# bryanlimy/tf2-cyclegan

Hardware: AMD Instinct MI355X
Metric: images/sec (whole node) horse2zebra 256×256 (higher is better)
Workload: dtype bf16; 1 GPU; model=cyclegan-resnet9-patchgan, global_batch=4, per_gpu_batch=4, image_size=256, parallelism=dp1

## Files before the change

cyclegan_amd/ops/_hip/bind.cpp:

```cpp
#include <torch/extension.h>

namespace cyg {
at::Tensor conv2d_fwd(at::Tensor, at::Tensor, c10::optional<at::Tensor>,
                      int64_t, int64_t, int64_t, int64_t, int64_t, bool,
                      int64_t, double);
at::Tensor convt2d_fwd(at::Tensor, at::Tensor, c10::optional<at::Tensor>,
                       int64_t, int64_t, int64_t, int64_t, int64_t, int64_t,
                       double);
std::vector<at::Tensor> conv2d_fwd_stats(at::Tensor, at::Tensor,
                                         c10::optional<at::Tensor>, int64_t,
                                         int64_t, int64_t, int64_t, int64_t,
                                         bool, int64_t, double);
std::vector<at::Tensor> convt2d_fwd_stats(at::Tensor, at::Tensor,
                                          c10::optional<at::Tensor>, int64_t,
                                          int64_t, int64_t, int64_t, int64_t,
                                          int64_t, double);
at::Tensor conv2d_dgrad(at::Tensor, at::Tensor, int64_t, int64_t, int64_t,
                        int64_t, int64_t, int64_t, int64_t, bool);
at::Tensor convt2d_dgrad(at::Tensor, at::Tensor, int64_t, int64_t, int64_t,
                         int64_t, int64_t);
at::Tensor conv2d_wgrad(at::Tensor, at::Tensor, int64_t, int64_t, int64_t,
                        int64_t, int64_t, bool);
void conv2d_wgrad_into(at::Tensor, at::Tensor, int64_t, int64_t, int64_t,
                       int64_t, int64_t, bool, at::Tensor, bool, bool);
void fold_packed_dw_into(at::Tensor, at::Tensor, bool);
at::Tensor mfma_probe(at::Tensor, at::Tensor);
at::Tensor mx_probe(at::Tensor, at::Tensor, int64_t, int64_t);
at::Tensor mx_probe16(at::Tensor, at::Tensor, int64_t, int64_t);
at::Tensor glds_probe(at::Tensor, at::Tensor);
at::Tensor tr_probe(int64_t);
at::Tensor quant_fp8(at::Tensor, at::Tensor);
at::Tensor quant_fp8_d(at::Tensor, at::Tensor, at::Tensor);
void amax_roll(at::Tensor, int64_t);
at::Tensor conv2d_fp8_fwd(at::Tensor, at::Tensor, at::Tensor,
                          c10::optional<at::Tensor>, c10::optional<at::Tensor>,
                          int64_t, int64_t, int64_t, int64_t, int64_t, bool, int64_t, double);
std::vector<at::Tensor> conv2d_fp8_fwd_stats(
    at::Tensor, at::Tensor, at::Tensor, c10::optional<at::Tensor>,
    c10::optional<at::Tensor>, int64_t, int64_t, int64_t, int64_t, int64_t,
    bool, int64_t, double);
std::vector<at::Tensor> instnorm_fwd(at::Tensor, at::Tensor, at::Tensor,
                                     double, int64_t, double,
                                     c10::optional<at::Tensor>,
                                     c10::optional<at::Tensor>,
                                     c10::optional<at::Tensor>, int64_t);
std::vector<at::Tensor> instnorm_fwd_q8(at::Tensor, at::Tensor, at::Tensor,
                                        double, int64_t, double,
                                        c10::optional<at::Tensor>,
                                        c10::optional<at::Tensor>,
                                        c10::optional<at::Tensor>, int64_t,
                                        at::Tensor, at::Tensor);
std::vector<at::Tensor> instnorm_bwd(at::Tensor, at::Tensor, at::Tensor,
                                     at::Tensor, at::Tensor,
                                     c10::optional<at::Tensor>, int64_t,
                                     double, c10::optional<at::Tensor>,
                                     c10::optional<at::Tensor>,
                                     c10::optional<at::Tensor>, bool);
at::Tensor act_bwd(at::Tensor, at::Tensor, int64_t, double);
at::Tensor channel_sum(at::Tensor, c10::optional<at::Tensor>, bool);
at::Tensor reflect_pad_fwd(at::Tensor, int64_t, int64_t, int64_t, int64_t);
at::Tensor reflect_pad_bwd(at::Tensor, int64_t, int64_t, int64_t, int64_t);
at::Tensor persample_loss_fwd(at::Tensor, at::Tensor, bool);
at::Tensor persample_loss_const_fwd(at::Tensor, double, bool);
std::vector<at::Tensor> persample_loss_bwd(at::Tensor, at::Tensor, at::Tensor,
                                           bool, bool, bool);
at::Tensor persample_loss_const_bwd(at::Tensor, double, at::Tensor, bool);
void adam_step_dev(at::Tensor, at::Tensor, at::Tensor, at::Tensor, at::Tensor,
                   double, double, double);
void adam_ema_step(at::Tensor, at::Tensor, at::Tensor, at::Tensor, at::Tensor,
                   double, double, double, double, int64_t, double);
void adam_ema_step_dev(at::Tensor, at::Tensor, at::Tensor, at::Tensor,
                       at::Tensor, at::Tensor, double, double, double, double);
void shadow_gather(at::Tensor, at::Tensor, at::Tensor);
void shadow_fold(at::Tensor, at::Tensor, at::Tensor);
void fold_upconv_dw_into(at::Tensor, at::Tensor, bool, bool);
void adam_step(at::Tensor, at::Tensor, at::Tensor, at::Tensor, double, double,
               double, double, int64_t);
at::Tensor augment_batch(at::Tensor, at::Tensor, at::Tensor, int64_t, int64_t,
                         at::Tensor);
at::Tensor pool_exchange(at::Tensor, at::Tensor, at::Tensor, at::Tensor);
std::vector<at::Tensor> ssim_fwd(at::Tensor, at::Tensor, int64_t);
at::Tensor ssim_bwd(at::Tensor, at::Tensor, at::Tensor, at::Tensor, at::Tensor,
                    at::Tensor);
}

PYBIND11_MODULE(TORCH_EXTENSION_NAME, m) {
  m.def("conv2d_fwd", &cyg::conv2d_fwd);
  m.def("convt2d_fwd", &cyg::convt2d_fwd);
  m.def("conv2d_fwd_stats", &cyg::conv2d_fwd_stats);
  m.def("convt2d_fwd_stats", &cyg::convt2d_fwd_stats);
  m.def("conv2d_dgrad", &cyg::conv2d_dgrad);
  m.def("convt2d_dgrad", &cyg::convt2d_dgrad);
  m.def("conv2d_wgrad", &cyg::conv2d_wgrad);
  m.def("conv2d_wgrad_into", &cyg::conv2d_wgrad_into, py::arg("x"),
        py::arg("dy"), py::arg("kh"), py::arg("kw"), py::arg("stride"),
        py::arg("pt"), py::arg("pl"), py::arg("reflect"), py::arg("out"),
        py::arg("accumulate"), py::arg("transpose_oi") = false);
  m.def("fold_packed_dw_into", &cyg::fold_packed_dw_into, py::arg("dwp"),
        py::arg("out"), py::arg("accumulate"));
  m.def("mfma_probe", &cyg::mfma_probe);
  m.def("mx_probe", &cyg::mx_probe);
  m.def("mx_probe16", &cyg::mx_probe16);
  m.def("glds_probe", &cyg::glds_probe);
  m.def("tr_probe", &cyg::tr_probe);
  m.def("quant_fp8", &cyg::quant_fp8);
  m.def("quant_fp8_d", &cyg::quant_fp8_d);
  m.def("amax_roll", &cyg::amax_roll);
  m.def("conv2d_fp8_fwd", &cyg::conv2d_fp8_fwd);
  m.def("conv2d_fp8_fwd_stats", &cyg::conv2d_fp8_fwd_stats);
  m.def("instnorm_fwd", &cyg::instnorm_fwd, py::arg("x"), py::arg("gamma"),
        py::arg("beta"), py::arg("eps"), py::arg("act"), py::arg("slope"),
        py::arg("residual"), py::arg("psum") = py::none(),
        py::arg("psq") = py::none(), py::arg("nslabs") = 0);
  m.def("instnorm_fwd_q8", &cyg::instnorm_fwd_q8, py::arg("x"),
        py::arg("gamma"), py::arg("beta"), py::arg("eps"), py::arg("act"),
        py::arg("slope"), py::arg("residual"), py::arg("psum"),
        py::arg("psq"), py::arg("nslabs"), py::arg("amax_prev"),
        py::arg("amax_cur"));
  m.def("instnorm_bwd", &cyg::instnorm_bwd, py::arg("dy"), py::arg("x"),
        py::arg("gamma"), py::arg("mean"), py::arg("rstd"), py::arg("yact"),
        py::arg("act"), py::arg("slope"), py::arg("beta") = py::none(),
        py::arg("dgamma_out") = py::none(), py::arg("dbeta_out") = py::none(),
        py::arg("accumulate") = false);
  m.def("act_bwd", &cyg::act_bwd);
  m.def("channel_sum", &cyg::channel_sum, py::arg("x"),
        py::arg("out") = py::none(), py::arg("accumulate") = false);
  m.def("reflect_pad_fwd", &cyg::reflect_pad_fwd);
  m.def("reflect_pad_bwd", &cyg::reflect_pad_bwd);
  m.def("persample_loss_fwd", &cyg::persample_loss_fwd);
  m.def("persample_loss_const_fwd", &cyg::persample_loss_const_fwd);
  m.def("persample_loss_bwd", &cyg::persample_loss_bwd);
  m.def("persample_loss_const_bwd", &cyg::persample_loss_const_bwd);
  m.def("adam_step", &cyg::adam_step);
  m.def("adam_step_dev", &cyg::adam_step_dev);
  m.def("adam_ema_step", &cyg::adam_ema_step);
  m.def("adam_ema_step_dev", &cyg::adam_ema_step_dev);
  m.def("shadow_gather", &cyg::shadow_gather);
  m.def("shadow_fold", &cyg::shadow_fold);
  m.def("fold_upconv_dw_into", &cyg::fold_upconv_dw_into, py::arg("dv"),
        py::arg("out"), py::arg("accumulate"), py::arg("transposed"));
  m.def("augment_batch", &cyg::augment_batch);
  m.def("pool_exchange", &cyg::pool_exchange);
  m.def("ssim_fwd", &cyg::ssim_fwd, py::arg("y_true"), py::arg("y_pred"),
        py::arg("save_maps") = 0);
  m.def("ssim_bwd", &cyg::ssim_bwd, py::arg("x"), py::arg("y"), py::arg("am"),
        py::arg("bm"), py::arg("cm"), py::arg("dout"));
}
```

cyclegan_amd/ops/_hip/conv.hip:

```cpp

#include <torch/extension.h>
#include <ATen/cuda/CUDAContext.h>

#include "common.h"

namespace cyg {

constexpr int BM = 128, BN = 64, BK = 64;
constexpr int NTHREADS = 256;
constexpr int LDK = BK + 8;

struct ConvParams {
  const short* __restrict__ x;
  const short* __restrict__ w;
  const short* __restrict__ bias;
  short* __restrict__ y;
  int B, H, W, Cin, OH, OW, Cout, KH, KW;
  int stride, pt, pl;
  int reflect;
  int act;  float slope;
  const float* dq;
  const float* dqb;
  long M, KTOT;
  int mtiles, ntiles;
  float* psum;
  float* psq;
  int tps;
  long ringoff;
  int wt, wl, wH, wW;
};

DEV int ring_index(int qh, int qw, int OH, int OW, int wt, int wl, int wH,
                   int wW) {
  if (qh < wt) return qh * OW + qw;
  if (qh >= wt + wH) return (qh - wH) * OW + qw;
  return (OH - wH) * OW + (qh - wt) * (OW - wW) + (qw < wl ? qw : qw - wW);
}

DEV int xcd_chunk(int bid, int nb) {
  return (nb % 8 == 0) ? (bid % 8) * (nb / 8) + bid / 8 : bid;
}


template <bool IS_CONVT, bool ALIGNED, int STRIDE>
__global__ __launch_bounds__(NTHREADS) void conv_gemm_kernel(ConvParams p) {
  const int stride = STRIDE ? STRIDE : p.stride;
  __shared__ short As[BM][LDK];
  __shared__ short Bs[BN][LDK];
  __shared__ long rowxb[BM];
  __shared__ long rowyb[BM];
  __shared__ int rowih[BM], rowiw[BM];
  __shared__ char rowok[BM];

  const int tid = threadIdx.x;
  const int lane = tid & 63;
  const int wid = tid >> 6;
  const int bid = xcd_chunk(blockIdx.x, gridDim.x);
  const int mt = bid % p.mtiles, nt = bid / p.mtiles;
  const long m0 = (long)mt * BM;
  const int n0 = nt * BN;

  for (int r = tid; r < BM; r += NTHREADS) {
    long m = m0 + r;
    bool ok = m < p.M;
    long mm = ok ? m : 0;
    int ow = (int)(mm % p.OW);
    int oh = (int)((mm / p.OW) % p.OH);
    int b = (int)(mm / ((long)p.OW * p.OH));
    rowok[r] = ok;
    rowxb[r] = (long)b * p.H * p.W * p.Cin;
    rowyb[r] = ((long)(b * p.OH + oh) * p.OW + ow) * p.Cout;
    if (IS_CONVT) {
      rowih[r] = oh + p.pt;
      rowiw[r] = ow + p.pl;
    } else {
      rowih[r] = oh * stride - p.pt;
      rowiw[r] = ow * stride - p.pl;
    }
  }
  __syncthreads();

  v4f acc[4][2] = {};

  const int wr = wid >> 1, wc = wid & 1;
  const int wm0 = wr * 64, wn0 = wc * 32;
  const int fr = lane & 15;
  const int fg = lane >> 4;

  for (long k0 = 0; k0 < p.KTOT; k0 += BK) {
    if (ALIGNED) {
      #pragma unroll 2
      for (int c = tid; c < BM * (BK / 8); c += NTHREADS) {
        int row = c >> 3;
        int kc = (c & 7) * 8;
        long k = k0 + kc;
        v8s val = {};
        if (k < p.KTOT && rowok[row]) {
          int tap = (int)(k / p.Cin);
          int ci = (int)(k - (long)tap * p.Cin);
          int dkh = tap / p.KW, dkw = tap - (tap / p.KW) * p.KW;
          bool valid = true;
          int ih, iw;
          if (IS_CONVT) {
            int nh = rowih[row] - dkh, nw = rowiw[row] - dkw;
            valid = nh >= 0 && nw >= 0 && (nh % stride) == 0 &&
                    (nw % stride) == 0;
            ih = nh / stride; iw = nw / stride;
            valid = valid && ih < p.H && iw < p.W;
          } else {
            ih = rowih[row] + dkh; iw = rowiw[row] + dkw;
            if (p.reflect) {
              ih = mirror_idx(ih, p.H); iw = mirror_idx(iw, p.W);
            } else {
              valid = ih >= 0 && ih < p.H && iw >= 0 && iw < p.W;
            }
          }
          if (valid)
            val = *(const v8s*)(p.x + rowxb[row] + ((long)ih * p.W + iw) * p.Cin + ci);
        }
        *(v8s*)&As[row][kc] = val;
// ... 25 lines not shown
            }
          }
          if (valid)
            val = p.x[rowxb[row] + ((long)ih * p.W + iw) * p.Cin + ci];
        }
        As[row][kc] = val;
      }
    }

    if (ALIGNED) {
      #pragma unroll 2
      for (int c = tid; c < BN * (BK / 8); c += NTHREADS) {
        int n = c >> 3;
        int kc = (c & 7) * 8;
        long k = k0 + kc;
        v8s val = {};
        if (n0 + n < p.Cout && k < p.KTOT)
          val = *(const v8s*)(p.w + (long)(n0 + n) * p.KTOT + k);
        *(v8s*)&Bs[n][kc] = val;
      }
    } else {
      for (int c = tid; c < BN * BK; c += NTHREADS) {
        int n = c >> 6;
        int kc = c & 63;
        long k = k0 + kc;
        Bs[n][kc] = (n0 + n < p.Cout && k < p.KTOT)
                        ? p.w[(long)(n0 + n) * p.KTOT + k] : (short)0;
      }
    }
    __syncthreads();

    #pragma unroll
    for (int kk = 0; kk < BK; kk += 32) {
      v8bf a0 = *(const v8bf*)&As[wm0 + 0 * 16 + fr][kk + fg * 8];
      v8bf a1 = *(const v8bf*)&As[wm0 + 1 * 16 + fr][kk + fg * 8];
      v8bf a2 = *(const v8bf*)&As[wm0 + 2 * 16 + fr][kk + fg * 8];
      v8bf a3 = *(const v8bf*)&As[wm0 + 3 * 16 + fr][kk + fg * 8];
      v8bf b0 = *(const v8bf*)&Bs[wn0 + 0 * 16 + fr][kk + fg * 8];
      v8bf b1 = *(const v8bf*)&Bs[wn0 + 1 * 16 + fr][kk + fg * 8];
      acc[0][0] = __builtin_amdgcn_mfma_f32_16x16x32_bf16(a0, b0, acc[0][0], 0, 0, 0);
      acc[0][1] = __builtin_amdgcn_mfma_f32_16x16x32_bf16(a0, b1, acc[0][1], 0, 0, 0);
      acc[1][0] = __builtin_amdgcn_mfma_f32_16x16x32_bf16(a1, b0, acc[1][0], 0, 0, 0);
      acc[1][1] = __builtin_amdgcn_mfma_f32_16x16x32_bf16(a1, b1, acc[1][1], 0, 0, 0);
      acc[2][0] = __builtin_amdgcn_mfma_f32_16x16x32_bf16(a2, b0, acc[2][0], 0, 0, 0);
      acc[2][1] = __builtin_amdgcn_mfma_f32_16x16x32_bf16(a2, b1, acc[2][1], 0, 0, 0);
      acc[3][0] = __builtin_amdgcn_mfma_f32_16x16x32_bf16(a3, b0, acc[3][0], 0, 0, 0);
      acc[3][1] = __builtin_amdgcn_mfma_f32_16x16x32_bf16(a3, b1, acc[3][1], 0, 0, 0);
    }
    __syncthreads();
  }

  #pragma unroll
  for (int nf = 0; nf < 2; ++nf) {
    int n = n0 + wn0 + nf * 16 + fr;
    if (n >= p.Cout) continue;
    float bv = p.bias ? b2f(p.bias[n]) : 0.f;
    #pragma unroll
    for (int mf = 0; mf < 4; ++mf) {
      #pragma unroll
      for (int r = 0; r < 4; ++r) {
        int rl = wm0 + mf * 16 + fg * 4 + r;
        if (!rowok[rl]) continue;
        float v = apply_act(acc[mf][nf][r] + bv, p.act, p.slope);
        p.y[rowyb[rl] + n] = f2b(v);
      }
    }
  }
}


template <int BNT>
struct ConvSmemT {
  long rowyb[BM];
  int rowih[BM], rowiw[BM];
  unsigned rowxb[BM];
  char rowok[BM];
  char _pad[16 - (BM % 16 ? BM % 16 : 16)];
  short A[2][BM * BK];
  short Bt[2][BNT * BK];
};

constexpr int NW = 8;

template <bool IS_CONVT, int STRIDE, int BNT, bool PHASED = false>
__global__ __launch_bounds__(NW * 64) void conv_glds_kernel(ConvParams p) {
  constexpr int NT = NW * 64;
  constexpr int API = 16 / NW;
  constexpr int TBI = BNT / 8;
  constexpr int BPI = TBI >= NW ? TBI / NW : 1;
  constexpr int NF = BNT >= 32 ? 2 : 1;
  constexpr int NWC = BNT / (NF * 16);
  constexpr int NWR = NW / NWC;
  constexpr int MF = (BM / NWR) / 16;
  const int stride = STRIDE ? STRIDE : p.stride;
  extern __shared__ __attribute__((aligned(16))) char smem_raw[];
  auto& sm = *reinterpret_cast<ConvSmemT<BNT>*>(smem_raw);

  const int tid = threadIdx.x;
  const int lane = tid & 63;
  const int w = tid >> 6;
  const int bid = (IS_CONVT && STRIDE == 2)
                      ? blockIdx.x : xcd_chunk(blockIdx.x, gridDim.x);
  const int mt = bid % p.mtiles, nt = bid / p.mtiles;
  const int n0 = nt * BNT;

  static_assert(!PHASED || (IS_CONVT && STRIDE == 2), "PHASED");
  const int tpp = PHASED ? (p.mtiles >> 2) : 0;
  const int phase = PHASED ? mt / tpp : 0;
  const int phh = phase >> 1, phw = phase & 1;
  const int OH2 = p.OH >> 1, OW2 = p.OW >> 1;
  const long m0 = PHASED ? (long)(mt - phase * tpp) * BM : (long)mt * BM;
  const int nvh = PHASED ? ((p.KH - phh + 1) >> 1) : 0;
  const int nvw = PHASED ? ((p.KW - phw + 1) >> 1) : 0;
  const long KEFF = PHASED ? (long)nvh * nvw * p.Cin : p.KTOT;

  for (int r = tid; r < BM; r += NT) {
    if (PHASED) {
      long mp = m0 + r;
      long Mp = (long)p.B * OH2 * OW2;
      bool ok = mp < Mp;
      long mm = ok ? mp : 0;
      int owp = (int)(mm % OW2);
      int ohp = (int)((mm / OW2) % OH2);
      int b = (int)(mm / ((long)OW2 * OH2));
      int i = 2 * ohp + ((phh + p.pt) & 1);
      int j = 2 * owp + ((phw + p.pl) & 1);
      sm.rowok[r] = ok && i < p.OH && j < p.OW;
      sm.rowxb[r] = (unsigned)((long)b * p.H * p.W * p.Cin * 2);
      sm.rowyb[r] = ((long)(b * p.OH + i) * p.OW + j) * p.Cout;
      sm.rowih[r] = (i + p.pt - phh) >> 1;
      sm.rowiw[r] = (j + p.pl - phw) >> 1;
    } else {
      long m = m0 + r;
      bool ok = m < p.M;
      long mm = ok ? m : 0;
      int ow = (int)(mm % p.OW);
      int oh = (int)((mm / p.OW) % p.OH);
      int b = (int)(mm / ((long)p.OW * p.OH));
      sm.rowok[r] = ok;
      sm.rowxb[r] = (unsigned)((long)b * p.H * p.W * p.Cin * 2);
      long yb = ((long)(b * p.OH + oh) * p.OW + ow) * p.Cout;
      if (IS_CONVT && p.ringoff != 0) {
        const int i = oh - p.wt, j = ow - p.wl;
        if ((unsigned)i < (unsigned)p.wH && (unsigned)j < (unsigned)p.wW) {
          yb = (((long)b * p.wH + i) * p.wW + j) * p.Cout;
        } else {
          const long rp = (long)p.OH * p.OW - (long)p.wH * p.wW;
          yb = p.ringoff +
               (b * rp + ring_index(oh, ow, p.OH, p.OW, p.wt, p.wl, p.wH,
                                    p.wW)) * p.Cout;
        }
      }
      sm.rowyb[r] = yb;
      if (IS_CONVT) {
        sm.rowih[r] = oh + p.pt;
        sm.rowiw[r] = ow + p.pl;
      } else {
        sm.rowih[r] = oh * stride - p.pt;
        sm.rowiw[r] = ow * stride - p.pl;
      }
    }
  }
  __syncthreads();

  const int lr = lane >> 3;
  const int klog = ((lane & 7) ^ lr) << 3;
  int aih[API], aiw[API];
  unsigned axb[API];
  bool aok[API];
  #pragma unroll
  for (int j = 0; j < API; ++j) {
    int r = (w * API + j) * 8 + lr;
    aih[j] = sm.rowih[r];
    aiw[j] = sm.rowiw[r];
    axb[j] = sm.rowxb[r];
    aok[j] = sm.rowok[r];
  }
  int bn[BPI];
  #pragma unroll
  for (int j = 0; j < BPI; ++j) bn[j] = (w * BPI + j) * 8 + lr + n0;
  const bool bw_on = w * BPI < TBI;
  static_assert(BNT == 16 || BNT == 64 || BNT == 128, "BNT");

  auto rx = __builtin_amdgcn_make_buffer_rsrc(
      (void*)p.x, 0, (unsigned)((long)p.B * p.H * p.W * p.Cin * 2), 0x00020000);
  auto rw = __builtin_amdgcn_make_buffer_rsrc(
      (void*)p.w, 0, (unsigned)(p.Cout * p.KTOT * 2), 0x00020000);

  const int nk = (int)((KEFF + BK - 1) / BK);
  const bool big_ci = p.Cin >= BK;

  long kcur;
  bool kv;
  int ci, dkh, dkw;
  unsigned avo[API];
  bool avalid[API];
  unsigned bvo[BPI];
  bool bnv[BPI];

  auto recompute_a = [&]() {
    #pragma unroll
    for (int j = 0; j < API; ++j) {
      avalid[j] = false;
      avo[j] = 0xFF000000u;
      if (!aok[j]) continue;
      bool valid = true;
      int ih, iw;
      if (PHASED) {
        ih = aih[j] - dkh; iw = aiw[j] - dkw;
        valid = ih >= 0 && iw >= 0 && ih < p.H && iw < p.W;
      } else if (IS_CONVT) {
        int nh = aih[j] - dkh, nw = aiw[j] - dkw;
        valid = nh >= 0 && nw >= 0 && (nh % stride) == 0 && (nw % stride) == 0;
        ih = nh / stride; iw = nw / stride;
        valid = valid && ih < p.H && iw < p.W;
      } else {
        ih = aih[j] + dkh; iw = aiw[j] + dkw;
        if (p.reflect) {
          ih = mirror_idx(ih, p.H); iw = mirror_idx(iw, p.W);
        } else {
          valid = ih >= 0 && ih < p.H && iw >= 0 && iw < p.W;
        }
      }
      if (valid) {
        avalid[j] = true;
        avo[j] = axb[j] + (unsigned)((((long)ih * p.W + iw) * p.Cin + ci) * 2);
      }
    }
  };

  auto recompute_b = [&]() {
    long kw_idx = kcur;
    if (PHASED)
      kw_idx = ((long)(2 * dkh + phh) * p.KW + (2 * dkw + phw)) * p.Cin + ci;
    #pragma unroll
    for (int j = 0; j < BPI; ++j)
      bvo[j] = (unsigned)(((long)bn[j] * p.KTOT + kw_idx) * 2);
  };

  auto decode_tap = [&]() {
    int tap = (int)(kcur / p.Cin);
    ci = (int)(kcur - (long)tap * p.Cin);
    if (PHASED) {
      dkh = tap / nvw;
      dkw = tap - dkh * nvw;
    } else {
      dkh = tap / p.KW;
      dkw = tap - dkh * p.KW;
    }
  };

  auto init_state = [&]() {
    kcur = klog;
    kv = kcur < KEFF;
    decode_tap();
    recompute_a();
    #pragma unroll
    for (int j = 0; j < BPI; ++j) bnv[j] = bn[j] < p.Cout;
    recompute_b();
  };

  auto advance = [&]() {
    kcur += BK;
    kv = kcur < KEFF;
    if (big_ci) {
      ci += BK;
      if (ci >= p.Cin) {
        ci -= p.Cin;
        if (PHASED) {
          if (++dkw == nvw) { dkw = 0; ++dkh; }
        } else {
          if (++dkw == p.KW) { dkw = 0; ++dkh; }
        }
        recompute_a();
        recompute_b();
      } else {
        #pragma unroll
        for (int j = 0; j < API; ++j) avo[j] += BK * 2;
        #pragma unroll
        for (int j = 0; j < BPI; ++j) bvo[j] += BK * 2;
      }
    } else {
      decode_tap();
      recompute_a();
      recompute_b();
    }
  };

  auto stage = [&](int buf) {
    #pragma unroll
    for (int j = 0; j < API; ++j) {
      unsigned vo = (kv && avalid[j]) ? avo[j] : 0xFF000000u;
      __builtin_amdgcn_raw_ptr_buffer_load_lds(
          rx, (__attribute__((address_space(3))) void*)&sm.A[buf][(w * API + j) * 512],
          16, vo, 0, 0, 0);
    }
    if (bw_on) {
      #pragma unroll
      for (int j = 0; j < BPI; ++j) {
        unsigned vo = (kv && bnv[j]) ? bvo[j] : 0xFF000000u;
        __builtin_amdgcn_raw_ptr_buffer_load_lds(
            rw, (__attribute__((address_space(3))) void*)&sm.Bt[buf][(w * BPI + j) * 512],
            16, vo, 0, 0, 0);
      }
    }
  };

  v4f acc[MF][NF] = {};
  const int wr = w / NWC, wc = w % NWC;
  const int wm0 = wr * (MF * 16), wn0 = wc * (NF * 16);
  const int fr = lane & 15;
  const int fg = lane >> 4;
  const int swz = (fr & 7) << 4;

  init_state();
  stage(0);
  __syncthreads();

  for (int kt = 0; kt < nk; ++kt) {
    if (kt + 1 < nk) {
      advance();
      stage((kt + 1) & 1);
    }
    const char* Ab = (const char*)sm.A[kt & 1];
    const char* Bb = (const char*)sm.Bt[kt & 1];
    #pragma unroll
    for (int kk = 0; kk < BK; kk += 32) {
      const int kbyte = (kk + fg * 8) * 2;
      v8bf a[MF], b[NF];
      #pragma unroll
      for (int mf = 0; mf < MF; ++mf)
        a[mf] = *(const v8bf*)(Ab + ((wm0 + mf * 16 + fr) << 7) + (kbyte ^ swz));
      #pragma unroll
      for (int nf = 0; nf < NF; ++nf)
        b[nf] = *(const v8bf*)(Bb + ((wn0 + nf * 16 + fr) << 7) + (kbyte ^ swz));
      #pragma unroll
      for (int mf = 0; mf < MF; ++mf)
        #pragma unroll
        for (int nf = 0; nf < NF; ++nf)
          acc[mf][nf] = __builtin_amdgcn_mfma_f32_16x16x32_bf16(
              a[mf], b[nf], acc[mf][nf], 0, 0, 0);
    }
    __syncthreads();
  }

  float cs[NF] = {}, cq[NF] = {};
  #pragma unroll
  for (int nf = 0; nf < NF; ++nf) {
    int n = n0 + wn0 + nf * 16 + fr;
    if (n >= p.Cout) continue;
    float bv = p.bias ? b2f(p.bias[n]) : 0.f;
    #pragma unroll
    for (int mf = 0; mf < MF; ++mf) {
      #pragma unroll
      for (int r = 0; r < 4; ++r) {
        int rl = wm0 + mf * 16 + fg * 4 + r;
// ... 1064 lines not shown
  if (q < nr * W) {
    i = span_nth(rs, q / W);
    j = q % W;
  } else {
    q -= nr * W;
    i = span_nth_out(rs, q / nc);
    j = span_nth(cs, q % nc);
  }
  int HP = H + pt + pb, WP = W + pl + pr;
  long rp = (long)HP * WP - (long)H * W;
  short* own = dx + (((long)b * H + i) * W + j) * C + g * 8;
  float s[8] = {};
  int hc[3] = {pt + i, pt - i, pt + 2 * (H - 1) - i};
  int wc_[3] = {pl + j, pl - j, pl + 2 * (W - 1) - j};
  #pragma unroll
  for (int a = 0; a < 3; ++a) {
    int qh = hc[a];
    if (qh < 0 || qh >= HP) continue;
    if (a > 0 && qh == hc[0]) continue;
    if (a == 2 && qh == hc[1]) continue;
    if (mirror_idx(qh - pt, H) != i) continue;
    #pragma unroll
    for (int d = 0; d < 3; ++d) {
      int qw = wc_[d];
      if (qw < 0 || qw >= WP) continue;
      if (d > 0 && qw == wc_[0]) continue;
      if (d == 2 && qw == wc_[1]) continue;
      if (mirror_idx(qw - pl, W) != j) continue;
      const short* src = (a == 0 && d == 0)
          ? own
          : ring + (b * rp + ring_index(qh, qw, HP, WP, pt, pl, H, W)) * C +
                g * 8;
      v8s v = *(const v8s*)src;
      #pragma unroll
      for (int e = 0; e < 8; ++e) s[e] += b2f(v[e]);
    }
  }
  v8s out;
  #pragma unroll
  for (int e = 0; e < 8; ++e) out[e] = f2b(s[e]);
  *(v8s*)own = out;
}


static inline int cdiv(long a, long b) { return (int)((a + b - 1) / b); }

static inline bool env_flag(const char* v) { return v && v[0] == '1'; }

static Span2 mirror_span(int n, int lo, int hi) {
  const int a0 = 1, b0 = std::min(lo, n - 1);
  const int a1 = std::max(n - 1 - hi, 0), b1 = n - 2;
  const int n0 = std::max(b0 - a0 + 1, 0), n1 = std::max(b1 - a1 + 1, 0);
  if (n0 == 0) return {a1, n1, a1 + n1, 0};
  if (n1 == 0) return {a0, n0, a0 + n0, 0};
  if (a1 <= a0 + n0) {
    const int a = std::min(a0, a1), b = std::max(b0, b1);
    return {a, b - a + 1, b + 1, 0};
  }
  return {a0, n0, a1, n1};
}

template <bool IS_CONVT, bool ALIGNED>
static void launch_conv_s(const ConvParams& p, dim3 grid, hipStream_t stream) {
  switch (p.stride) {
    case 1:
      hipLaunchKernelGGL((conv_gemm_kernel<IS_CONVT, ALIGNED, 1>), grid,
                         dim3(NTHREADS), 0, stream, p);
      break;
    case 2:
      hipLaunchKernelGGL((conv_gemm_kernel<IS_CONVT, ALIGNED, 2>), grid,
                         dim3(NTHREADS), 0, stream, p);
      break;
    default:
      hipLaunchKernelGGL((conv_gemm_kernel<IS_CONVT, ALIGNED, 0>), grid,
                         dim3(NTHREADS), 0, stream, p);
  }
}

static int conv_ntile(int Cout) {
  if (Cout <= 16) return 16;
  return (Cout % 128) == 0 ? 128 : 64;
}

template <bool IS_CONVT, int STRIDE, int BNT, bool PHASED = false>
static void launch_one_glds(const ConvParams& p, hipStream_t stream) {
  constexpr size_t SMB = sizeof(ConvSmemT<BNT>);
  static bool init = []() {
    hipFuncSetAttribute(
        (const void*)(conv_glds_kernel<IS_CONVT, STRIDE, BNT, PHASED>),
        hipFuncAttributeMaxDynamicSharedMemorySize, (int)SMB);
    return true;
  }();
  (void)init;
  hipLaunchKernelGGL((conv_glds_kernel<IS_CONVT, STRIDE, BNT, PHASED>),
                     dim3((long)p.mtiles * p.ntiles), dim3(NW * 64), SMB,
                     stream, p);
  hipError_t err = hipGetLastError();
  TORCH_CHECK(err == hipSuccess, "conv_glds launch failed (BNT=", BNT,
              " PHASED=", PHASED, "): ", hipGetErrorString(err));
}

template <bool IS_CONVT, int BNT>
static void launch_glds_s(const ConvParams& p, hipStream_t stream) {
  switch (p.stride) {
    case 1: launch_one_glds<IS_CONVT, 1, BNT>(p, stream); break;
    case 2: launch_one_glds<IS_CONVT, 2, BNT>(p, stream); break;
    default: launch_one_glds<IS_CONVT, 0, BNT>(p, stream);
  }
}

template <bool IS_CONVT>
static void launch_glds(ConvParams p, hipStream_t stream) {
  const int bnt = conv_ntile(p.Cout);
  p.ntiles = cdiv(p.Cout, bnt);
  switch (bnt) {
    case 16: launch_glds_s<IS_CONVT, 16>(p, stream); break;
    case 128: launch_glds_s<IS_CONVT, 128>(p, stream); break;
    default: launch_glds_s<IS_CONVT, 64>(p, stream);
  }
}

static bool glds_eligible(const ConvParams& p) {
  return (p.Cin % 8) == 0 &&
         (long)p.B * p.H * p.W * p.Cin * 2 < (1L << 31) &&
         (long)p.Cout * p.KTOT * 2 < (1L << 31);
}

static bool phased_eligible(const ConvParams& p, bool is_convt) {
  return glds_eligible(p) && is_convt && p.stride == 2 && (p.OH % 2) == 0 &&
         (p.OW % 2) == 0;
}

static int stats_cap() {
  static const int cap = []() {
    const char* off = getenv("CYG_NO_CONV_STATS");
    if (off && off[0] == '1') return 0;
    const char* e = getenv("CYG_CONV_STATS_MAXSLABS");
    return e ? atoi(e) : 128;
  }();
  return cap;
}

static int stats_slabs(const ConvParams& p, bool is_convt, bool fp8,
                       int* tps) {
  const int cap = stats_cap();
  if (cap <= 0 || p.Cout <= 16 || (p.Cout % 8) != 0) return 0;
  if (!fp8 && !glds_eligible(p)) return 0;
  const bool phased = !fp8 && phased_eligible(p, is_convt);
  const long per = phased ? (long)(p.OH / 2) * (p.OW / 2)
                          : (long)p.OH * p.OW;
  const long ns = (phased ? 4 : 1) * (per / BM);
  if (per % BM != 0 || ns > cap) return 0;
  *tps = (int)(per / BM);
  return (int)ns;
}

static void launch_conv(const ConvParams& p, bool is_convt, hipStream_t stream) {
  if (phased_eligible(p, is_convt)) {
    ConvParams q = p;
    long Mp = (long)q.B * (q.OH / 2) * (q.OW / 2);
    q.mtiles = 4 * cdiv(Mp, BM);
    if (conv_ntile(q.Cout) == 128) {
      q.ntiles = cdiv(q.Cout, 128);
      launch_one_glds<true, 2, 128, true>(q, stream);
    } else {
      launch_one_glds<true, 2, 64, true>(q, stream);
    }
    return;
  }
  if (glds_eligible(p)) {
    if (is_convt) launch_glds<true>(p, stream);
    else launch_glds<false>(p, stream);
    return;
  }
  dim3 grid(p.mtiles * p.ntiles);
  bool aligned = (p.Cin % 8) == 0;
  if (is_convt) {
    if (aligned) launch_conv_s<true, true>(p, grid, stream);
    else launch_conv_s<true, false>(p, grid, stream);
  } else {
    if (aligned) launch_conv_s<false, true>(p, grid, stream);
    else launch_conv_s<false, false>(p, grid, stream);
// ... 51 lines not shown
  launch_conv(p, is_convt, at::cuda::getCurrentCUDAStream());
  return out;
}

static std::vector<at::Tensor> conv2d_fwd_impl(
    at::Tensor x, at::Tensor w, c10::optional<at::Tensor> bias,
    int64_t stride, int64_t pt, int64_t pb, int64_t pl, int64_t pr,
    bool reflect, int64_t act, double slope, bool want_stats) {
  check_conv_inputs(x, w);
  int H = x.size(1), W = x.size(2);
  int KH = w.size(1), KW = w.size(2);
  int OH = (H + pt + pb - KH) / stride + 1;
  int OW = (W + pl + pr - KW) / stride + 1;
  auto y = at::empty({x.size(0), OH, OW, w.size(0)}, x.options());
  auto p = fill_common(x, w, bias, y, stride, act, slope);
  p.pt = pt; p.pl = pl; p.reflect = reflect ? 1 : 0;
  return run_fwd(p, y, false, want_stats);
}

static std::vector<at::Tensor> convt2d_fwd_impl(
    at::Tensor x, at::Tensor w, c10::optional<at::Tensor> bias,
    int64_t stride, int64_t pt, int64_t pl, int64_t out_h, int64_t out_w,
    int64_t act, double slope, bool want_stats) {
  check_conv_inputs(x, w);
  auto y = at::empty({x.size(0), out_h, out_w, w.size(0)}, x.options());
  auto p = fill_common(x, w, bias, y, stride, act, slope);
  p.pt = pt; p.pl = pl; p.reflect = 0;
  return run_fwd(p, y, true, want_stats);
}

at::Tensor conv2d_fwd(at::Tensor x, at::Tensor w, c10::optional<at::Tensor> bias,
                      int64_t stride, int64_t pt, int64_t pb, int64_t pl,
                      int64_t pr, bool reflect, int64_t act, double slope) {
  return conv2d_fwd_impl(x, w, bias, stride, pt, pb, pl, pr, reflect, act,
                         slope, false)[0];
}

std::vector<at::Tensor> conv2d_fwd_stats(
    at::Tensor x, at::Tensor w, c10::optional<at::Tensor> bias,
    int64_t stride, int64_t pt, int64_t pb, int64_t pl, int64_t pr,
    bool reflect, int64_t act, double slope) {
  return conv2d_fwd_impl(x, w, bias, stride, pt, pb, pl, pr, reflect, act,
                         slope, true);
}

at::Tensor convt2d_fwd(at::Tensor x, at::Tensor w, c10::optional<at::Tensor> bias,
                       int64_t stride, int64_t pt, int64_t pl,
                       int64_t out_h, int64_t out_w, int64_t act, double slope) {
  return convt2d_fwd_impl(x, w, bias, stride, pt, pl, out_h, out_w, act,
                          slope, false)[0];
}

std::vector<at::Tensor> convt2d_fwd_stats(
    at::Tensor x, at::Tensor w, c10::optional<at::Tensor> bias,
    int64_t stride, int64_t pt, int64_t pl, int64_t out_h, int64_t out_w,
    int64_t act, double slope) {
  return convt2d_fwd_impl(x, w, bias, stride, pt, pl, out_h, out_w, act,
                          slope, true);
}

at::Tensor conv2d_dgrad(at::Tensor dy, at::Tensor wt, int64_t H, int64_t W,
                        int64_t stride, int64_t pt, int64_t pb, int64_t pl,
                        int64_t pr, bool reflect) {
  check_conv_inputs(dy, wt);
  auto stream = at::cuda::getCurrentCUDAStream();
  if (!reflect) {
    auto dx = at::empty({dy.size(0), H, W, wt.size(0)}, dy.options());
    auto p = fill_common(dy, wt, c10::nullopt, dx, stride, ACT_NONE, 0.0);
    p.pt = pt; p.pl = pl;
    launch_conv(p, true, stream);
    return dx;
  }
  TORCH_CHECK(wt.size(0) % 8 == 0, "reflect dgrad: Cin % 8 != 0");
  long HP = H + pt + pb, WP = W + pl + pr;
  const long B = dy.size(0), C = wt.size(0);
  const long nimg = B * H * W * C;
  auto dxp = at::empty({B, HP, WP, C}, dy.options());
  auto p = fill_common(dy, wt, c10::nullopt, dxp, stride, ACT_NONE, 0.0);
  p.pt = 0; p.pl = 0;
  int threads = 256;
  if (stride == 1 && HP * WP > H * W && glds_eligible(p) &&
      !env_flag(getenv("CYG_NO_DIRECT_FOLD"))) {
    auto dx = dxp.view({-1}).narrow(0, 0, nimg).view({B, H, W, C});
    p.ringoff = nimg;
    p.wt = pt; p.wl = pl; p.wH = H; p.wW = W;
    launch_conv(p, true, stream);
    const Span2 rs = mirror_span(H, pt, pb), cs = mirror_span(W, pl, pr);
    const long nr = rs.n0 + rs.n1, nc = cs.n0 + cs.n1;
    const long total = B * (nr * W + (H - nr) * nc) * (C / 8);
    if (total > 0)
      hipLaunchKernelGGL(reflect_ring_add_kernel, dim3(cdiv(total, threads)),
                         dim3(threads), 0, stream, p.y, p.y + nimg, (int)B,
                         (int)H, (int)W, (int)C, (int)pt, (int)pb, (int)pl,
                         (int)pr, rs, cs);
    return dx;
  }
  launch_conv(p, true, stream);
  auto dx = at::empty({B, H, W, C}, dy.options());
  long total = dx.numel() / 8;
  hipLaunchKernelGGL(reflect_fold_kernel, dim3(cdiv(total, threads)),
                     dim3(threads), 0, stream,
                     (const short*)dxp.const_data_ptr(),
                     (short*)dx.mutable_data_ptr(),
                     (int)dy.size(0), (int)H, (int)W, (int)wt.size(0),
                     (int)pt, (int)pb, (int)pl, (int)pr);
  return dx;
}

at::Tensor convt2d_dgrad(at::Tensor dy, at::Tensor wt, int64_t IH, int64_t IW,
                         int64_t stride, int64_t pt, int64_t pl) {
  check_conv_inputs(dy, wt);
  int KH = wt.size(1), KW = wt.size(2);
  auto dx = at::empty({dy.size(0), IH, IW, wt.size(0)}, dy.options());
  auto p = fill_common(dy, wt, c10::nullopt, dx, stride, ACT_NONE, 0.0);
  p.pt = pt; p.pl = pl; p.reflect = 0;
  launch_conv(p, false, at::cuda::getCurrentCUDAStream());
  return dx;
}

struct WgSplit { int slices; long mchunks_per_slice; };
static WgSplit wgrad_split(long M, int ktiles, int ntiles) {
  static const int tgt_blocks = []() {
    const char* e = getenv("CYG_WG_BLOCKS");
    return e ? atoi(e) : 512;
  }();
  const long mchunks = (M + WG_BM - 1) / WG_BM;
  const int target = std::max<long>(1, tgt_blocks / ((long)ktiles * ntiles));
  const int slices = (int)std::min<long>(mchunks, target);
  const long per = (mchunks + slices - 1) / slices;
  return {(int)((mchunks + per - 1) / per), per};
}

template <int WBN>
static void launch_wgrad_glds(const WgradParams& p, dim3 grid,
                              hipStream_t stream) {
  constexpr size_t SMB = sizeof(WgSmemT<WBN>);
  if constexpr (WBN == 128) {
    static bool init = []() {
      hipFuncSetAttribute((const void*)(wgrad_glds_kernel<128>),
                          hipFuncAttributeMaxDynamicSharedMemorySize,
                          (int)SMB);
      return true;
    }();
    (void)init;
  }
  hipLaunchKernelGGL((wgrad_glds_kernel<WBN>), grid, dim3(NW * 64), SMB,
                     stream, p);
}

static at::Tensor wgrad_impl(at::Tensor x, at::Tensor dy, int64_t KH,
                             int64_t KW, int64_t stride, int64_t pt,
                             int64_t pl, bool reflect, const at::Tensor* into,
                             bool accumulate, bool transpose_oi) {
  TORCH_CHECK(x.is_cuda() && dy.is_cuda() && x.is_contiguous() && dy.is_contiguous());
  TORCH_CHECK(x.scalar_type() == at::kBFloat16 && dy.scalar_type() == at::kBFloat16);
  TORCH_CHECK(dy.size(0) == x.size(0));
  WgradParams p{};
  p.x = (const short*)x.const_data_ptr();
  p.dy = (const short*)dy.const_data_ptr();
  p.B = x.size(0); p.H = x.size(1); p.W = x.size(2); p.Cin = x.size(3);
  p.OH = dy.size(1); p.OW = dy.size(2); p.Cout = dy.size(3);
  p.KH = KH; p.KW = KW; p.stride = stride; p.pt = pt; p.pl = pl;
  p.reflect = reflect ? 1 : 0;
  p.M = (long)p.B * p.OH * p.OW;
  p.KTOT = (long)KH * KW * p.Cin;
  const bool glds_ok = (p.Cin % 8) == 0 && (p.Cout % 8) == 0 &&
                       (long)p.B * p.H * p.W * p.Cin * 2 < (1L << 31) &&
                       p.M * p.Cout * 2 < (1L << 31);
  const int wbn = glds_ok ? conv_ntile(p.Cout) : WG_BN;
  p.ktiles = cdiv(p.KTOT, WG_BK);
  p.ntiles = cdiv(p.Cout, wbn);
  const WgSplit split = wgrad_split(p.M, p.ktiles, p.ntiles);
  p.slices = split.slices;
  p.mchunks_per_slice = split.mchunks_per_slice;
  dim3 grid((long)p.ktiles * p.ntiles * p.slices);
  auto stream = at::cuda::getCurrentCUDAStream();
  if (!glds_ok) {
    auto dw = at::zeros({p.Cout, (long)KH, (long)KW, p.Cin},
                        x.options().dtype(at::kFloat));
    p.dw = (float*)dw.mutable_data_ptr();
    hipLaunchKernelGGL(wgrad_kernel, grid, dim3(NTHREADS), 0, stream, p);
    if (!into) return dw;
    auto v = transpose_oi ? dw.permute({3, 1, 2, 0}) : dw;
    v = v.narrow(0, 0, into->size(0)).narrow(3, 0, into->size(3));
    if (accumulate) into->add_(v); else into->copy_(v);
    return *into;
  }
  at::Tensor dw;
  if (!into) {
// ... 180 lines not shown
```

Baseline: 350.6 images/s.

## Reorder reflect-pad dgrad tiles by region and trim out-of-range kernel taps

The reflect-padded stride-1 dgrad, which writes into an interior plus ring layout, now uses a dedicated RING kernel variant. Output rows are grouped into interior tiles and four border-strip classes (top, bottom, left, right), and each border tile loops only over the kernel taps that can touch it. This skips multiply-accumulates on taps that would only read zero-padded dy. It adds per-tile class decoding, a separate block-to-tile mapping, and a host-side rowmap debugging function, and adds complexity to the kernel's index math.

Result: faster. 356.6 images/s, median of 6 (+1.7%).

```diff
diff --git a/cyclegan_amd/ops/_hip/bind.cpp b/cyclegan_amd/ops/_hip/bind.cpp
--- a/cyclegan_amd/ops/_hip/bind.cpp
+++ b/cyclegan_amd/ops/_hip/bind.cpp
@@ -17,6 +17,9 @@
                                           int64_t, double);
 at::Tensor conv2d_dgrad(at::Tensor, at::Tensor, int64_t, int64_t, int64_t,
                         int64_t, int64_t, int64_t, int64_t, bool);
+at::Tensor reflect_dgrad_rowmap(int64_t, int64_t, int64_t, int64_t, int64_t,
+                                int64_t, int64_t, int64_t, int64_t, bool,
+                                bool);
 at::Tensor convt2d_dgrad(at::Tensor, at::Tensor, int64_t, int64_t, int64_t,
                          int64_t, int64_t);
 at::Tensor conv2d_wgrad(at::Tensor, at::Tensor, int64_t, int64_t, int64_t,
@@ -90,6 +93,10 @@
   m.def("conv2d_fwd_stats", &cyg::conv2d_fwd_stats);
   m.def("convt2d_fwd_stats", &cyg::convt2d_fwd_stats);
   m.def("conv2d_dgrad", &cyg::conv2d_dgrad);
+  m.def("reflect_dgrad_rowmap", &cyg::reflect_dgrad_rowmap, py::arg("B"),
+        py::arg("H"), py::arg("W"), py::arg("pt"), py::arg("pb"),
+        py::arg("pl"), py::arg("pr"), py::arg("KH"), py::arg("KW"),
+        py::arg("trim") = true, py::arg("frame") = false);
   m.def("convt2d_dgrad", &cyg::convt2d_dgrad);
   m.def("conv2d_wgrad", &cyg::conv2d_wgrad);
   m.def("conv2d_wgrad_into", &cyg::conv2d_wgrad_into, py::arg("x"),
diff --git a/cyclegan_amd/ops/_hip/conv.hip b/cyclegan_amd/ops/_hip/conv.hip
--- a/cyclegan_amd/ops/_hip/conv.hip
+++ b/cyclegan_amd/ops/_hip/conv.hip
@@ -9,6 +9,88 @@
 constexpr int BM = 128, BN = 64, BK = 64;
 constexpr int NTHREADS = 256;
 constexpr int LDK = BK + 8;
+
+#define HDEV __host__ __device__ __forceinline__
+
+HDEV int ring_index(int qh, int qw, int OH, int OW, int wt, int wl, int wH,
+                    int wW) {
+  if (qh < wt) return qh * OW + qw;
+  if (qh >= wt + wH) return (qh - wH) * OW + qw;
+  return (OH - wH) * OW + (qh - wt) * (OW - wW) + (qw < wl ? qw : qw - wW);
+}
+
+struct ReflectOrder {
+  int B, H, W;
+  int pt, pb, pl, pr;
+  int KH, KW;
+  int frame;
+  int trim;
+  int wtiles;
+  int cstart[5];
+  int crows[4];
+};
+
+struct TapWindow { int kh0, kh1, kw0, kw1; };
+HDEV TapWindow reflect_taps(const ReflectOrder& o, int cls) {
+  TapWindow t = {0, o.KH, 0, o.KW};
+  if (!o.trim) return t;
+  if (cls == 1) t.kh1 = o.pt < o.KH ? o.pt : o.KH;
+  if (cls == 2) t.kh0 = o.KH > o.pb ? o.KH - o.pb : 0;
+  if (cls == 3) t.kw1 = o.pl < o.KW ? o.pl : o.KW;
+  if (cls == 4) t.kw0 = o.KW > o.pr ? o.KW - o.pr : 0;
+  return t;
+}
+
+HDEV int reflect_tile_class(const ReflectOrder& o, int tile) {
+  if (tile < o.wtiles) return 0;
+  return 1 + (tile >= o.cstart[1]) + (tile >= o.cstart[2]) +
+         (tile >= o.cstart[3]);
+}
+
+struct ReflectRow {
+  int ok, b, qh, qw, cls;
+  TapWindow taps;
+  long dst;
+};
+HDEV ReflectRow reflect_row(const ReflectOrder& o, int tile, int r) {
+  const int HP = o.pt + o.H + o.pb, WP = o.pl + o.W + o.pr;
+  ReflectRow d;
+  d.cls = reflect_tile_class(o, tile);
+  d.taps = reflect_taps(o, d.cls);
+  if (d.cls == 0) {
+    const long m = (long)tile * BM + r;
+    const int fh = o.frame ? HP : o.H, fw = o.frame ? WP : o.W;
+    d.ok = m < (long)o.B * fh * fw;
+    const long mm = d.ok ? m : 0;
+    d.qw = (int)(mm % fw) + (o.frame ? 0 : o.pl);
+    d.qh = (int)((mm / fw) % fh) + (o.frame ? 0 : o.pt);
+    d.b = (int)(mm / ((long)fw * fh));
+  } else {
+    const int c = d.cls;
+    const int start = c == 1 ? o.cstart[0] : c == 2 ? o.cstart[1]
+                    : c == 3 ? o.cstart[2] : o.cstart[3];
+    const int rows = c == 1 ? o.crows[0] : c == 2 ? o.crows[1]
+                   : c == 3 ? o.crows[2] : o.crows[3];
+    const int wide = c <= 2 ? WP : c == 3 ? o.pl : o.pr;
+    const int x = (tile - start) * BM + r;
+    d.ok = x < rows;
+    const int xx = d.ok ? x : 0;
+    const int per = rows / o.B;
+    d.b = xx / per;
+    const int rem = xx - d.b * per;
+    d.qh = rem / wide + (c == 1 ? 0 : c == 2 ? o.pt + o.H : o.pt);
+    d.qw = rem % wide + (c == 4 ? o.pl + o.W : 0);
+  }
+  const int i = d.qh - o.pt, j = d.qw - o.pl;
+  if ((unsigned)i < (unsigned)o.H && (unsigned)j < (unsigned)o.W) {
+    d.dst = ((long)d.b * o.H + i) * o.W + j;
+  } else {
+    const long rp = (long)HP * WP - (long)o.H * o.W;
+    d.dst = (long)o.B * o.H * o.W + d.b * rp +
+            ring_index(d.qh, d.qw, HP, WP, o.pt, o.pl, o.H, o.W);
+  }
+  return d;
+}
 
 struct ConvParams {
   const short* __restrict__ x;
@@ -26,16 +108,8 @@
   float* psum;
   float* psq;
   int tps;
-  long ringoff;
-  int wt, wl, wH, wW;
+  ReflectOrder ro;
 };
-
-DEV int ring_index(int qh, int qw, int OH, int OW, int wt, int wl, int wH,
-                   int wW) {
-  if (qh < wt) return qh * OW + qw;
-  if (qh >= wt + wH) return (qh - wH) * OW + qw;
-  return (OH - wH) * OW + (qh - wt) * (OW - wW) + (qw < wl ? qw : qw - wW);
-}
 
 DEV int xcd_chunk(int bid, int nb) {
   return (nb % 8 == 0) ? (bid % 8) * (nb / 8) + bid / 8 : bid;
@@ -227,7 +301,8 @@
 
 constexpr int NW = 8;
 
-template <bool IS_CONVT, int STRIDE, int BNT, bool PHASED = false>
+template <bool IS_CONVT, int STRIDE, int BNT, bool PHASED = false,
+          bool RING = false>
 __global__ __launch_bounds__(NW * 64) void conv_glds_kernel(ConvParams p) {
   constexpr int NT = NW * 64;
   constexpr int API = 16 / NW;
@@ -244,9 +319,23 @@
   const int tid = threadIdx.x;
   const int lane = tid & 63;
   const int w = tid >> 6;
-  const int bid = (IS_CONVT && STRIDE == 2)
-                      ? blockIdx.x : xcd_chunk(blockIdx.x, gridDim.x);
-  const int mt = bid % p.mtiles, nt = bid / p.mtiles;
+  int mt, nt;
+  if (RING) {
+    static_assert(!RING || (IS_CONVT && STRIDE == 1 && !PHASED), "RING");
+    const int nbw = p.ro.wtiles * p.ntiles;
+    const int rb = (int)blockIdx.x - nbw;
+    if (rb < 0) {
+      const int bid = xcd_chunk(blockIdx.x, nbw);
+      mt = bid % p.ro.wtiles; nt = bid / p.ro.wtiles;
+    } else {
+      const int rt = p.mtiles - p.ro.wtiles;
+      mt = p.ro.wtiles + rb % rt; nt = rb / rt;
+    }
+  } else {
+    const int bid = (IS_CONVT && STRIDE == 2)
+                        ? blockIdx.x : xcd_chunk(blockIdx.x, gridDim.x);
+    mt = bid % p.mtiles; nt = bid / p.mtiles;
+  }
   const int n0 = nt * BNT;
 
   static_assert(!PHASED || (IS_CONVT && STRIDE == 2), "PHASED");
@@ -257,10 +346,22 @@
   const long m0 = PHASED ? (long)(mt - phase * tpp) * BM : (long)mt * BM;
   const int nvh = PHASED ? ((p.KH - phh + 1) >> 1) : 0;
   const int nvw = PHASED ? ((p.KW - phw + 1) >> 1) : 0;
-  const long KEFF = PHASED ? (long)nvh * nvw * p.Cin : p.KTOT;
+  const TapWindow tw =
+      RING ? reflect_taps(p.ro, reflect_tile_class(p.ro, mt)) : TapWindow{};
+  const int nkw = RING ? tw.kw1 - tw.kw0 : 0;
+  const long KEFF = PHASED ? (long)nvh * nvw * p.Cin
+                  : RING ? (long)(tw.kh1 - tw.kh0) * nkw * p.Cin : p.KTOT;
+  const int tapw = PHASED ? nvw : RING ? nkw : p.KW;
 
   for (int r = tid; r < BM; r += NT) {
-    if (PHASED) {
+    if (RING) {
+      const ReflectRow d = reflect_row(p.ro, mt, r);
+      sm.rowok[r] = d.ok;
+      sm.rowxb[r] = (unsigned)((long)d.b * p.H * p.W * p.Cin * 2);
+      sm.rowyb[r] = d.dst * p.Cout;
+      sm.rowih[r] = d.qh + p.pt - tw.kh0;
+      sm.rowiw[r] = d.qw + p.pl - tw.kw0;
+    } else if (PHASED) {
       long mp = m0 + r;
       long Mp = (long)p.B * OH2 * OW2;
       bool ok = mp < Mp;
@@ -284,19 +385,7 @@
       int b = (int)(mm / ((long)p.OW * p.OH));
       sm.rowok[r] = ok;
       sm.rowxb[r] = (unsigned)((long)b * p.H * p.W * p.Cin * 2);
-      long yb = ((long)(b * p.OH + oh) * p.OW + ow) * p.Cout;
-      if (IS_CONVT && p.ringoff != 0) {
-        const int i = oh - p.wt, j = ow - p.wl;
-        if ((unsigned)i < (unsigned)p.wH && (unsigned)j < (unsigned)p.wW) {
-          yb = (((long)b * p.wH + i) * p.wW + j) * p.Cout;
-        } else {
-          const long rp = (long)p.OH * p.OW - (long)p.wH * p.wW;
-          yb = p.ringoff +
-               (b * rp + ring_index(oh, ow, p.OH, p.OW, p.wt, p.wl, p.wH,
-                                    p.wW)) * p.Cout;
-        }
-      }
-      sm.rowyb[r] = yb;
+      sm.rowyb[r] = ((long)(b * p.OH + oh) * p.OW + ow) * p.Cout;
       if (IS_CONVT) {
         sm.rowih[r] = oh + p.pt;
         sm.rowiw[r] = ow + p.pl;
@@ -327,10 +416,14 @@
   const bool bw_on = w * BPI < TBI;
   static_assert(BNT == 16 || BNT == 64 || BNT == 128, "BNT");
 
-  auto rx = __builtin_amdgcn_make_buffer_rsrc(
-      (void*)p.x, 0, (unsigned)((long)p.B * p.H * p.W * p.Cin * 2), 0x00020000);
-  auto rw = __builtin_amdgcn_make_buffer_rsrc(
-      (void*)p.w, 0, (unsigned)(p.Cout * p.KTOT * 2), 0x00020000);
+  unsigned xbytes = (unsigned)((long)p.B * p.H * p.W * p.Cin * 2);
+  unsigned wbytes = (unsigned)(p.Cout * p.KTOT * 2);
+  if (RING) {
+    xbytes = __builtin_amdgcn_readfirstlane(xbytes);
+    wbytes = __builtin_amdgcn_readfirstlane(wbytes);
+  }
+  auto rx = __builtin_amdgcn_make_buffer_rsrc((void*)p.x, 0, xbytes, 0x00020000);
+  auto rw = __builtin_amdgcn_make_buffer_rsrc((void*)p.w, 0, wbytes, 0x00020000);
 
   const int nk = (int)((KEFF + BK - 1) / BK);
   const bool big_ci = p.Cin >= BK;
@@ -378,6 +471,8 @@
     long kw_idx = kcur;
     if (PHASED)
       kw_idx = ((long)(2 * dkh + phh) * p.KW + (2 * dkw + phw)) * p.Cin + ci;
+    if (RING)
+      kw_idx = ((long)(tw.kh0 + dkh) * p.KW + (tw.kw0 + dkw)) * p.Cin + ci;
     #pragma unroll
     for (int j = 0; j < BPI; ++j)
       bvo[j] = (unsigned)(((long)bn[j] * p.KTOT + kw_idx) * 2);
@@ -386,13 +481,8 @@
   auto decode_tap = [&]() {
     int tap = (int)(kcur / p.Cin);
     ci = (int)(kcur - (long)tap * p.Cin);
-    if (PHASED) {
-      dkh = tap / nvw;
-      dkw = tap - dkh * nvw;
-    } else {
-      dkh = tap / p.KW;
-      dkw = tap - dkh * p.KW;
-    }
+    dkh = tap / tapw;
+    dkw = tap - dkh * tapw;
   };
 
   auto init_state = [&]() {
@@ -412,11 +502,7 @@
       ci += BK;
       if (ci >= p.Cin) {
         ci -= p.Cin;
-        if (PHASED) {
-          if (++dkw == nvw) { dkw = 0; ++dkh; }
-        } else {
-          if (++dkw == p.KW) { dkw = 0; ++dkh; }
-        }
+        if (++dkw == tapw) { dkw = 0; ++dkh; }
         recompute_a();
         recompute_b();
       } else {
@@ -1647,22 +1733,55 @@
   return (Cout % 128) == 0 ? 128 : 64;
 }
 
-template <bool IS_CONVT, int STRIDE, int BNT, bool PHASED = false>
+template <bool IS_CONVT, int STRIDE, int BNT, bool PHASED = false,
+          bool RING = false>
 static void launch_one_glds(const ConvParams& p, hipStream_t stream) {
   constexpr size_t SMB = sizeof(ConvSmemT<BNT>);
   static bool init = []() {
     hipFuncSetAttribute(
-        (const void*)(conv_glds_kernel<IS_CONVT, STRIDE, BNT, PHASED>),
+        (const void*)(conv_glds_kernel<IS_CONVT, STRIDE, BNT, PHASED, RING>),
         hipFuncAttributeMaxDynamicSharedMemorySize, (int)SMB);
     return true;
   }();
   (void)init;
-  hipLaunchKernelGGL((conv_glds_kernel<IS_CONVT, STRIDE, BNT, PHASED>),
+  hipLaunchKernelGGL((conv_glds_kernel<IS_CONVT, STRIDE, BNT, PHASED, RING>),
                      dim3((long)p.mtiles * p.ntiles), dim3(NW * 64), SMB,
                      stream, p);
   hipError_t err = hipGetLastError();
   TORCH_CHECK(err == hipSuccess, "conv_glds launch failed (BNT=", BNT,
-              " PHASED=", PHASED, "): ", hipGetErrorString(err));
+              " PHASED=", PHASED, " RING=", RING, "): ",
+              hipGetErrorString(err));
+}
+
+static ReflectOrder reflect_order(int B, int H, int W, int pt, int pb, int pl,
+                                  int pr, int KH, int KW, bool frame,
+                                  bool trim) {
+  ReflectOrder o{};
+  o.B = B; o.H = H; o.W = W;
+  o.pt = pt; o.pb = pb; o.pl = pl; o.pr = pr;
+  o.KH = KH; o.KW = KW;
+  o.frame = frame; o.trim = trim && !frame;
+  const long HP = H + pt + pb, WP = W + pl + pr;
+  o.wtiles = cdiv(frame ? B * HP * WP : (long)B * H * W, BM);
+  const long rows[4] = {B * pt * WP, B * pb * WP, (long)B * H * pl,
+                        (long)B * H * pr};
+  o.cstart[0] = o.wtiles;
+  for (int c = 0; c < 4; ++c) {
+    o.crows[c] = frame ? 0 : (int)rows[c];
+    o.cstart[c + 1] = o.cstart[c] + cdiv(o.crows[c], BM);
+  }
+  return o;
+}
+
+static void launch_ring(ConvParams p, hipStream_t stream) {
+  p.mtiles = p.ro.cstart[4];
+  if (conv_ntile(p.Cout) == 128) {
+    p.ntiles = cdiv(p.Cout, 128);
+    launch_one_glds<true, 1, 128, false, true>(p, stream);
+  } else {
+    p.ntiles = cdiv(p.Cout, 64);
+    launch_one_glds<true, 1, 64, false, true>(p, stream);
+  }
 }
 
 template <bool IS_CONVT, int BNT>
@@ -1880,9 +1999,13 @@
   if (stride == 1 && HP * WP > H * W && glds_eligible(p) &&
       !env_flag(getenv("CYG_NO_DIRECT_FOLD"))) {
     auto dx = dxp.view({-1}).narrow(0, 0, nimg).view({B, H, W, C});
-    p.ringoff = nimg;
-    p.wt = pt; p.wl = pl; p.wH = H; p.wW = W;
-    launch_conv(p, true, stream);
+    const int KH = wt.size(1), KW = wt.size(2);
+    TORCH_CHECK(dy.size(1) == HP - KH + 1 && dy.size(2) == WP - KW + 1,
+                "reflect dgrad: dy is not the stride-1 output frame");
+    p.ro = reflect_order(B, H, W, pt, pb, pl, pr, KH, KW,
+                         env_flag(getenv("CYG_DGRAD_FRAME_ORDER")),
+                         p.Cin % BK == 0);
+    launch_ring(p, stream);
     const Span2 rs = mirror_span(H, pt, pb), cs = mirror_span(W, pl, pr);
     const long nr = rs.n0 + rs.n1, nc = cs.n0 + cs.n1;
     const long total = B * (nr * W + (H - nr) * nc) * (C / 8);
@@ -1903,6 +2026,30 @@
                      (int)dy.size(0), (int)H, (int)W, (int)wt.size(0),
                      (int)pt, (int)pb, (int)pl, (int)pr);
   return dx;
+}
+
+at::Tensor reflect_dgrad_rowmap(int64_t B, int64_t H, int64_t W, int64_t pt,
+                                int64_t pb, int64_t pl, int64_t pr,
+                                int64_t KH, int64_t KW, bool trim,
+                                bool frame) {
+  TORCH_CHECK(B > 0 && H > 0 && W > 0 && KH > 0 && KW > 0 && pt >= 0 &&
+              pb >= 0 && pl >= 0 && pr >= 0, "reflect_dgrad_rowmap: sizes");
+  TORCH_CHECK(B * (H + pt + pb) * (W + pl + pr) < (1L << 24),
+              "reflect_dgrad_rowmap: a table for small shapes");
+  const ReflectOrder o =
+      reflect_order(B, H, W, pt, pb, pl, pr, KH, KW, frame, trim);
+  const int tiles = o.cstart[4];
+  auto out = at::empty({(long)tiles * BM, 10}, at::kInt);
+  int* t = out.data_ptr<int>();
+  for (int tile = 0; tile < tiles; ++tile)
+    for (int r = 0; r < BM; ++r, t += 10) {
+      const ReflectRow d = reflect_row(o, tile, r);
+      t[0] = d.ok; t[1] = d.b; t[2] = d.qh; t[3] = d.qw; t[4] = d.cls;
+      t[5] = d.taps.kh0; t[6] = d.taps.kh1;
+      t[7] = d.taps.kw0; t[8] = d.taps.kw1;
+      t[9] = (int)d.dst;
+    }
+  return out;
 }
 
 at::Tensor convt2d_dgrad(at::Tensor dy, at::Tensor wt, int64_t IH, int64_t IW,
```
